# SyamVangara/multigrid-petsc

Hardware: AMD Instinct MI355X
Metric: fp64 DOF-updates/sec per V-cycle at 1024^3 (higher is better)
Workload: dtype f64

## Files before the change

multigrid_petsc_amd/csrc/mgk_kernels3.hip:

```cpp
#include "mgk_dev.hpp"
#include <type_traits>

struct J3dArgs {
    const double *u, *b, *uc;
    double *out;
    int nx, ny, nxc, nyc;
    long rs, crs;
    int ntx, yc, nwaves, xcd, bous, plainst;
    double a0, a2, a3, a4, a6, dinv, scale;
    const double *ctab, *dtab;
    double *partials;
    double *rout;
};
template <bool PRO, bool ZG, bool NORM, bool TAB, int YC>
__global__ void __launch_bounds__(256) k_jacobi3_2d(const J3dArgs a) {
    using VT = V16<double>;
    const int lane = threadIdx.x & 63;
    int bid = blockIdx.x;
    if (a.xcd) bid = (bid & 7) * (gridDim.x >> 3) + (bid >> 3);
    const int wid = __builtin_amdgcn_readfirstlane(bid * 4 + (threadIdx.x >> 6));
    const int tx = wid % a.ntx, cy = wid / a.ntx;
    const int yc = YC > 0 ? YC : a.yc;
    const int y0 = cy * yc, y1 = min(y0 + yc, a.ny);
    if (y0 >= y1) { if (NORM && lane == 0) a.partials[wid] = 0.0; return; }
    const int pidx = tx * 60 + lane - 2;
    const int x0 = 2 * pidx;
    const bool xin = (x0 >= 0 && x0 < a.nx);
    const bool lastvec = (x0 + 2 > a.nx);
    const bool store = (lane >= 2 && lane <= 61 && xin);
    const int xc = min(max(x0, 0), a.nx - 1);
    const double *__restrict__ up_ = a.u + xc;
    const double *__restrict__ bp_ = a.b + xc;
    const double *__restrict__ cp_ = PRO ? a.uc + min(max(pidx, -1), a.nxc) : nullptr;
    double *__restrict__ op_ = a.out + x0;
    const VT Z = v16_zero<double>();
    const bool nts = a.plainst == 2 || (a.plainst == 0 && mgk_store_nt_2d(a.ny, a.rs));
    auto fix = [&](VT v, int y) -> VT {
        if (!xin || y < 0 || y >= a.ny) { v.v[0] = 0.0; v.v[1] = 0.0; }
        if (lastvec) v.v[1] = 0.0;
        return v;
    };
    auto ldraw = [&](int y) -> VT { return *reinterpret_cast<const VT *>(up_ + (long)min(max(y, -1), a.ny) * a.rs); };
    auto ldbraw = [&](int y) -> VT { return ldv_stream(bp_ + (long)min(max(y, 0), a.ny - 1) * a.rs, true); };
    auto ldc = [&](int ic) -> double { return PRO ? cp_[(long)min(max(ic, -1), a.nyc) * a.crs] : 0.0; };
    auto pA = [&](int y) { return (y & 1) ? (y - 1) >> 1 : (y >> 1) - 1; };
    auto pB = [&](int y) { return (y & 1) ? (y - 1) >> 1 : (y >> 1); };
    auto correct = [&](VT v, int y, double cA, double cB) -> VT {
        if (PRO) {
            const bool two = ((y & 1) == 0);
            const double wi = two ? 0.5 : 1.0;
            const double wh = wi * 0.5, w1 = wi * 1.0;
            const double mA = lane_up<true>(cA), mB = lane_up<true>(cB);
            double s0 = 0.0, s1 = 0.0;
            s0 += wh * mA; s0 += wh * cA; s1 += w1 * cA;
            if (two) { s0 += wh * mB; s0 += wh * cB; s1 += w1 * cB; }
            v.v[0] = v.v[0] + s0; v.v[1] = v.v[1] + s1;
        }
        return fix(v, y);
    };
    struct K6 { double k0, k2, k3, k4, k6, kd; };
    auto ldk = [&](int y) -> K6 {
        K6 k = {a.a0, a.a2, a.a3, a.a4, a.a6, a.dinv};
        if (TAB) {
            const int yy_ = min(max(y, 0), a.ny - 1);
            const CDBL4 *cr_ = (const CDBL4 *)(a.ctab + 5 * (long)yy_);
            const CDBL4 *dr_ = (const CDBL4 *)(a.dtab + yy_);
            k.k0 = cr_[0]; k.k2 = cr_[1]; k.k3 = cr_[2]; k.k4 = cr_[3]; k.k6 = cr_[4]; k.kd = dr_[0];
        }
        return k;
    };
#define J3_COEFS(kk)                                                                                                  \
    const double k0 = TAB ? (kk).k0 : a.a0, k2 = TAB ? (kk).k2 : a.a2, k3 = TAB ? (kk).k3 : a.a3, k4 = TAB ? (kk).k4 : a.a4,    \
                 k6 = TAB ? (kk).k6 : a.a6, kd = TAB ? (kk).kd : a.dinv;
    double nacc = 0.0;
    auto sweep = [&](const VT &lo, const VT &c, const VT &hi, const VT &bb, int y, bool norm, const K6 &kk) -> VT {
        J3_COEFS(kk)
        const double Wv = lane_up<true>(c.v[1]), Ev = lane_dn<true>(c.v[0]);
        VT o, rr;
#pragma unroll
        for (int e = 0; e < 2; e++) {
            const double wv = (e == 0) ? Wv : c.v[0];
            const double ev = (e == 1) ? Ev : c.v[1];
            double s = k0 * lo.v[e];
            s = s + k2 * wv;
            s = s + k3 * c.v[e];
            s = s + k4 * ev;
            s = s + k6 * hi.v[e];
            const double res = bb.v[e] - s;
            const double zz = res * kd;
            o.v[e] = c.v[e] + a.scale * zz;
            rr.v[e] = (lastvec && e == 1) ? 0.0 : res;
            if (NORM && norm) nacc += (store && y >= y0 && y < y1 && !(lastvec && e == 1)) ? res * res : 0.0;
        }
        if (NORM && norm && a.rout && store && y >= y0 && y < y1) stv_policy(a.rout + (long)y * a.rs + x0, rr, nts);
        return fix(o, y);
    };
    auto sweep0 = [&](const VT &bb, int y, const K6 &kk) -> VT {
        J3_COEFS(kk)
        (void)k0; (void)k2; (void)k3; (void)k4; (void)k6;
        VT o;
#pragma unroll
        for (int e = 0; e < 2; e++) { const double zz = bb.v[e] * kd; o.v[e] = a.scale * zz; }
        return fix(o, y);
    };
    VT UU[2] = {Z, Z};
    VT BB[3] = {Z, Z, Z};
    VT PP[2] = {Z, Z};
    VT QQ[2] = {Z, Z};
    auto stepg = [&](auto revc, const int K, int t, const VT &ur, double cA, double cB, const VT &bnext) {
        constexpr bool REV = decltype(revc)::value;
        auto ph = [&](int tt) -> int { return REV ? (y0 + y1 - 1 - tt) : tt; };
        const K6 kc2 = ldk(ph(t + 2)), kc1 = ldk(ph(t + 1)), kc0 = ldk(ph(t));
        VT &ua = UU[K & 1], &ub = UU[(K + 1) & 1];
        VT &p0 = PP[K & 1], &p1 = PP[(K + 1) & 1];
        VT &q0 = QQ[K & 1], &q1 = QQ[(K + 1) & 1];
        VT &b0 = BB[K % 3], &b1 = BB[(K + 1) % 3], &b2 = BB[(K + 2) % 3];
        VT p2;
        if (ZG) p2 = sweep0(b2, ph(t + 2), kc2);
        else {
            const VT uc = correct(ur, ph(t + 3), cA, cB);
            p2 = REV ? sweep(uc, ub, ua, b2, ph(t + 2), true, kc2) : sweep(ua, ub, uc, b2, ph(t + 2), true, kc2);
            ua = uc;
        }
        if (t >= y0 - 2) {
            const VT q2 = REV ? sweep(p2, p1, p0, b1, ph(t + 1), false, kc1) : sweep(p0, p1, p2, b1, ph(t + 1), false, kc1);
            if (t >= y0 && t < y1) {
                const VT o = REV ? sweep(q2, q1, q0, b0, ph(t), false, kc0) : sweep(q0, q1, q2, b0, ph(t), false, kc0);
                if (store) stv_policy(op_ + (long)ph(t) * a.rs, o, nts);
            }
            q0 = q2;
        }
        p0 = p2;
        b0 = fix(bnext, ph(t + 3));
    };
    const int t0 = y0 - 4;
    if constexpr (YC > 0) {
        constexpr int NU = YC + 6, NC = NU / 2 + 2;
        VT U[NU], B[NU];
        double Cc[NC];
        const int c0 = pA(t0 + 1);
#pragma unroll
        for (int q = 0; q < NU; q++) { if (!ZG) U[q] = ldraw(t0 + 1 + q); B[q] = ldbraw(t0 + 1 + q); }
#pragma unroll
        for (int q = 0; q < NC; q++) Cc[q] = ldc(c0 + q);
        if (!ZG) {
            UU[0] = correct(U[0], t0 + 1, Cc[0], Cc[0]);
            UU[1] = correct(U[1], t0 + 2, Cc[0], Cc[1]);
        }
        BB[2] = fix(B[1], t0 + 2);
#pragma unroll
        for (int sidx = 0; sidx < YC + 4; sidx++) {
            const int k = sidx + 3;
            const int ia = (k & 1) ? (k - 1) / 2 : k / 2 - 1;
            const int ib = (k & 1) ? (k - 1) / 2 : k / 2;
            stepg(std::false_type{}, sidx % 6, t0 + sidx, ZG ? Z : U[sidx + 2], Cc[ia], Cc[ib], B[sidx + 2]);
        }
    } else {
        auto march = [&](auto revc) {
            constexpr bool REV = decltype(revc)::value;
            auto ph = [&](int tt) -> int { return REV ? (y0 + y1 - 1 - tt) : tt; };
            VT UR[2] = {Z, Z}, BN[2];
            double CA[2] = {0.0, 0.0}, CB[2] = {0.0, 0.0};
            if (!ZG) {
                UU[0] = correct(ldraw(ph(t0 + 1)), ph(t0 + 1), ldc(pA(ph(t0 + 1))), ldc(pB(ph(t0 + 1))));
                UU[1] = correct(ldraw(ph(t0 + 2)), ph(t0 + 2), ldc(pA(ph(t0 + 2))), ldc(pB(ph(t0 + 2))));
                UR[0] = ldraw(ph(t0 + 3));
                CA[0] = ldc(pA(ph(t0 + 3))); CB[0] = ldc(pB(ph(t0 + 3)));
            }
            BB[2] = fix(ldbraw(ph(t0 + 2)), ph(t0 + 2));
            BN[0] = ldbraw(ph(t0 + 3));
            auto S = [&](const int K, int t) {
                if (!ZG) { UR[(K + 1) & 1] = ldraw(ph(t + 4)); CA[(K + 1) & 1] = ldc(pA(ph(t + 4))); CB[(K + 1) & 1] = ldc(pB(ph(t + 4))); }
                BN[(K + 1) & 1] = ldbraw(ph(t + 4));
                stepg(revc, K, t, UR[K & 1], CA[K & 1], CB[K & 1], BN[K & 1]);
            };
            int t = t0;
            for (; t + 6 <= y1; t += 6) { S(0, t); S(1, t + 1); S(2, t + 2); S(3, t + 3); S(4, t + 4); S(5, t + 5); }
            if (t < y1) { S(0, t); t++; }
            if (t < y1) { S(1, t); t++; }
            if (t < y1) { S(2, t); t++; }
            if (t < y1) { S(3, t); t++; }
            if (t < y1) { S(4, t); t++; }
        };
        if (a.bous && ((cy & 1) || a.bous == 2)) march(std::true_type{}); else march(std::false_type{});
    }
    if (NORM) {
        const double sw = wave_sum(nacc);
        if (lane == 0) a.partials[wid] = sw;
    }
#undef J3_COEFS
}
template <bool PRO, bool ZG, bool NORM>
static int jacobi3_2d(mgk_ctx *c, const mgk_geom *g, const mgk_geom *gc, const double *coef, double dinv, double scale, const double *ctab, const double *dtab,
                      const double *b, const double *uc, const double *u, double *unew, void *stream, int *norm_parts, double *rout = nullptr) {
    if (!c || !g || g->dim != 2 || (!coef && !ctab) || (ctab && !dtab) || !b || !unew || (!ZG && (!u || u == unew)) || b == unew)
        return fail(MGK_EINVAL, "mgk_jacobi3_2d: bad arguments (2-D)");
    J3dArgs a; memset(&a, 0, sizeof(a));
    a.u = ZG ? nullptr : u + g->org; a.b = b + g->org; a.out = unew + g->org;
    a.nx = g->nx; a.ny = g->ny; a.rs = g->pitch;
    if (PRO) {
        if (!gc || !uc || gc->dim != 2 || g->nx != 2 * gc->nx + 1 || g->ny != 2 * gc->ny + 1) return fail(MGK_EINVAL, "mgk_prolong_jacobi3_2d: coarse grid does not match");
        a.uc = uc + gc->org; a.nxc = gc->nx; a.nyc = gc->ny; a.crs = gc->pitch;
    }
    if (coef) { a.a0 = coef[0]; a.a2 = coef[1]; a.a3 = coef[2]; a.a4 = coef[3]; a.a6 = coef[4]; }
    a.dinv = dinv; a.scale = scale; a.ctab = ctab; a.dtab = dtab;
    if (rout) { if (!NORM || rout == unew || rout == u || rout == b) return fail(MGK_EINVAL, "mgk_jacobi3_2d_sumsq_store_f64: bad arguments"); a.rout = rout + g->org; }
    a.ntx = ((g->nx + 1) / 2 + 59) / 60;
    int ycs = (g->nx + 1 <= 1024) ? 4 : 0;
    if (g_variant == 50) ycs = 0; else if (g_variant == 51) ycs = 4; else if (g_variant == 52) ycs = 8;
    if (g_zchunk > 0 && g_variant != 51 && g_variant != 52) ycs = 0;
    long nch = (4096 + a.ntx - 1) / a.ntx;
    if (g_zchunk > 0) nch = (g->ny + g_zchunk - 1) / g_zchunk;
    int yc = (int)((g->ny + nch - 1) / nch);
    if (yc < 12 && g_zchunk <= 0) yc = 12;
    if (yc > g->ny) yc = g->ny;
    if (ycs) yc = ycs;
    long waves = (long)a.ntx * ((g->ny + yc - 1) / yc);
    if (NORM && ((waves + 3) / 4 + 7) * 4 > c->max_partials) {
        if (ycs) { ycs = 0; }
        const long maxch = c->max_partials / a.ntx - 1;
        if (maxch < 1) return fail(MGK_EINVAL, "mgk_jacobi3_2d_sumsq_f64: more waves than partial slots");
        yc = (int)((g->ny + maxch - 1) / maxch);
        waves = (long)a.ntx * ((g->ny + yc - 1) / yc);
    }
    a.yc = yc;
    unsigned nblk = (unsigned)((waves + 3) / 4);
    a.xcd = (g_variant == 54) || (g_variant != 53 && nblk >= 64 && (ycs != 0 || g->nx >= 4095));
    if (a.xcd) nblk = (nblk + 7u) & ~7u;
    a.nwaves = (int)waves;
    a.bous = (ycs == 0 && g_variant == 58) ? 1 : (ycs == 0 && g_variant == 59) ? 2 : 0;
    a.plainst = (g_variant == 60) ? 1 : (g_variant == 61) ? 2 : 0;
    if (NORM) {
        if (!norm_parts || 4L * nblk > c->max_partials) return fail(MGK_EINVAL, "mgk_jacobi3_2d_sumsq_f64: more waves than partial slots");
        a.partials = c->partials;
        *norm_parts = (int)(4 * nblk);
    }
    hipStream_t st = S(c, stream);
#define J3_LAUNCH(TABV, YCV) hipLaunchKernelGGL((k_jacobi3_2d<PRO, ZG, NORM, TABV, YCV>), dim3(nblk), dim3(256), 0, st, a)
    if (ctab) { if (ycs == 4) J3_LAUNCH(true, 4); else if (ycs == 8) J3_LAUNCH(true, 8); else J3_LAUNCH(true, 0); }
    else { if (ycs == 4) J3_LAUNCH(false, 4); else if (ycs == 8) J3_LAUNCH(false, 8); else J3_LAUNCH(false, 0); }
#undef J3_LAUNCH
    HIPCHK(hipGetLastError());
    return 0;
}
extern "C" int mgk_jacobi3_2d_f64(mgk_ctx *c, const mgk_geom *g, const double *coef, double dinv, double scale, const double *ctab, const double *dtab,
                                  const double *b, const double *u, double *unew, void *stream) {
    return jacobi3_2d<false, false, false>(c, g, nullptr, coef, dinv, scale, ctab, dtab, b, nullptr, u, unew, stream, nullptr);
}
extern "C" int mgk_jacobi3_2d_sumsq_f64(mgk_ctx *c, const mgk_geom *g, const double *coef, double dinv, double scale, const double *ctab, const double *dtab,
                                        const double *b, const double *u, double *unew, double *sumsq_host, void *stream) {
    if (!sumsq_host) return fail(MGK_EINVAL, "mgk_jacobi3_2d_sumsq_f64: bad arguments");
    int nparts = 0;
    int rc = jacobi3_2d<false, false, true>(c, g, nullptr, coef, dinv, scale, ctab, dtab, b, nullptr, u, unew, stream, &nparts);
    if (rc) return rc;
    return finish_to_host(c, nparts, 1, S(c, stream), sumsq_host);
}
extern "C" int mgk_jacobi3_2d_sumsq_store_f64(mgk_ctx *c, const mgk_geom *g, const double *coef, double dinv, double scale, const double *ctab, const double *dtab,
                                              const double *b, const double *u, double *unew, double *r, double *sumsq_host, void *stream) {
    if (!sumsq_host || !r) return fail(MGK_EINVAL, "mgk_jacobi3_2d_sumsq_store_f64: bad arguments");
    int nparts = 0;
    int rc = jacobi3_2d<false, false, true>(c, g, nullptr, coef, dinv, scale, ctab, dtab, b, nullptr, u, unew, stream, &nparts, r);
    if (rc) return rc;
    return finish_to_host(c, nparts, 1, S(c, stream), sumsq_host);
}
extern "C" int mgk_jacobi3_2d_zero_f64(mgk_ctx *c, const mgk_geom *g, const double *coef, double dinv, double scale, const double *ctab, const double *dtab,
                                       const double *b, double *unew, void *stream) {
    return jacobi3_2d<false, true, false>(c, g, nullptr, coef, dinv, scale, ctab, dtab, b, nullptr, nullptr, unew, stream, nullptr);
}
extern "C" int mgk_prolong_jacobi3_2d_f64(mgk_ctx *c, const mgk_geom *gf, const mgk_geom *gc, const double *coef, double dinv, double scale,
                                          const double *ctab, const double *dtab, const double *b, const double *uc, const double *u, double *unew, void *stream) {
    return jacobi3_2d<true, false, false>(c, gf, gc, coef, dinv, scale, ctab, dtab, b, uc, u, unew, stream, nullptr);
}

struct J33Args {
    const double *u, *b;
    double *out;
    int nx, ny, nz;
    long rs, ms;
    int ntx, nty, ntz, zc, xcd;
    double a0, a1, a2, a3, a4, a5, a6, dinv, scale;
    double *partials;
};
template <int TY, bool NORM, int g_form>
__global__ void __launch_bounds__(256, 1) k_jacobi3_3d(const J33Args a) {
    constexpr int R0 = TY + 6, R1 = TY + 4, R2 = TY + 2;
    using VT = V16<double>;
    const int lane = threadIdx.x & 63;
    int bid = blockIdx.x;
    if (a.xcd) bid = (bid & 7) * (gridDim.x >> 3) + (bid >> 3);
    const int wid = bid * 4 + __builtin_amdgcn_readfirstlane((int)(threadIdx.x >> 6));
    const int tx = wid % a.ntx, ty = (wid / a.ntx) % a.nty, tz = wid / (a.ntx * a.nty);
    const int z0 = tz * a.zc, z1 = min(z0 + a.zc, a.nz);
    if (tz >= a.ntz || z0 >= z1) { if (NORM && lane == 0) a.partials[wid] = 0.0; return; }
    const int yb = ty * TY;
    const int x0 = 2 * (tx * 60 + lane - 2);
    const bool xin = (x0 >= 0 && x0 < a.nx);
    const bool lastvec = (x0 + 2 > a.nx);
    const bool store = (lane >= 2 && lane <= 61 && xin);
    const unsigned lo = (unsigned)(8 * min(x0, a.nx + 1));
    const char *__restrict__ ub_ = reinterpret_cast<const char *>(a.u);
    const char *__restrict__ bb_ = reinterpret_cast<const char *>(a.b);
    char *__restrict__ ob_ = reinterpret_cast<char *>(a.out);
    const long loff = (long)(int)lo;
    const VT Z = v16_zero<double>();
    long uro[R0], bro[R1];
#pragma unroll
    for (int r = 0; r < R0; r++) uro[r] = 8 * (long)min(max(yb - 3 + r, -1), a.ny) * a.rs;
#pragma unroll
    for (int q = 0; q < R1; q++) bro[q] = 8 * (long)min(max(yb - 2 + q, 0), a.ny - 1) * a.rs;
    bool rowok[R1];
#pragma unroll
    for (int q = 0; q < R1; q++) rowok[q] = (yb - 2 + q >= 0 && yb - 2 + q < a.ny);
    double nacc = 0.0;
    const unsigned long long Mx0 = xin ? ~0ull : 0ull, Mx1 = (xin && !lastvec) ? ~0ull : 0ull;
    auto andm = [](double v, unsigned long long m) -> double { return __longlong_as_double((long long)((unsigned long long)__double_as_longlong(v) & m)); };
    auto jac = [&](const VT &dn, const VT &sv, const VT &c, const VT &nv, const VT &upv, const VT &bb, unsigned long long mu, bool own, bool norm) -> VT {
        const double Wv = lane_up<true>(c.v[1]), Ev = lane_dn<true>(c.v[0]);
        VT o;
#pragma unroll
        for (int e = 0; e < 2; e++) {
            const double wv = (e == 0) ? Wv : c.v[0];
            const double ev = (e == 1) ? Ev : c.v[1];
            double s = a.a0 * dn.v[e];
            s = s + a.a1 * sv.v[e];
            s = s + a.a2 * wv;
            s = s + a.a3 * c.v[e];
            s = s + a.a4 * ev;
            s = s + a.a5 * nv.v[e];
            s = s + a.a6 * upv.v[e];
            const double res = bb.v[e] - s;
            const double zz = res * a.dinv;
            const double val = c.v[e] + a.scale * zz;
            const unsigned long long m = (e == 0 ? Mx0 : Mx1) & mu;
            o.v[e] = andm(val, m);
            if (NORM && norm) { const double rm = andm(res, (own && store) ? m : 0ull); nacc += rm * rm; }
        }
        return o;
    };
    auto ldplane = [&](VT (&P)[R0], int z) {
        const char *pz = ub_ + 8 * (long)min(max(z, -1), a.nz) * a.ms + loff;
#pragma unroll
        for (int r = 0; r < R0; r++) P[r] = *reinterpret_cast<const VT *>(pz + uro[r]);
    };
    auto ldb = [&](VT (&P)[R1], int z) {
        const char *pz = bb_ + 8 * (long)min(max(z, 0), a.nz - 1) * a.ms + loff;
#pragma unroll
        for (int q = 0; q < R1; q++) P[q] = ldv_stream(reinterpret_cast<const double *>(pz + bro[q]), true);
    };
#define J33_STAGE(NR, OUT, DN, o_dn, C, UP, o_up, BB, o_b, MASK, ...)                                            \
    {                                                                                                                  \
        double s_[NR][2], w_[NR], e_[NR];                                                                              \
        _Pragma("unroll") for (int q = 0; q < NR; q++) { w_[q] = lane_up<true>(C[q + 1].v[1]); e_[q] = lane_dn<true>(C[q + 1].v[0]); } \
        _Pragma("unroll") for (int q = 0; q < NR; q++) { s_[q][0] = a.a0 * DN[q + o_dn].v[0]; s_[q][1] = a.a0 * DN[q + o_dn].v[1]; } \
        _Pragma("unroll") for (int q = 0; q < NR; q++) { s_[q][0] = s_[q][0] + a.a1 * C[q].v[0]; s_[q][1] = s_[q][1] + a.a1 * C[q].v[1]; } \
        _Pragma("unroll") for (int q = 0; q < NR; q++) { s_[q][0] = s_[q][0] + a.a2 * w_[q]; s_[q][1] = s_[q][1] + a.a2 * C[q + 1].v[0]; } \
        _Pragma("unroll") for (int q = 0; q < NR; q++) { s_[q][0] = s_[q][0] + a.a3 * C[q + 1].v[0]; s_[q][1] = s_[q][1] + a.a3 * C[q + 1].v[1]; } \
        _Pragma("unroll") for (int q = 0; q < NR; q++) { s_[q][0] = s_[q][0] + a.a4 * C[q + 1].v[1]; s_[q][1] = s_[q][1] + a.a4 * e_[q]; } \
        _Pragma("unroll") for (int q = 0; q < NR; q++) { s_[q][0] = s_[q][0] + a.a5 * C[q + 2].v[0]; s_[q][1] = s_[q][1] + a.a5 * C[q + 2].v[1]; } \
        _Pragma("unroll") for (int q = 0; q < NR; q++) { s_[q][0] = s_[q][0] + a.a6 * UP[q + o_up].v[0]; s_[q][1] = s_[q][1] + a.a6 * UP[q + o_up].v[1]; } \
        _Pragma("unroll") for (int q = 0; q < NR; q++) {                                                               \
            const double r0_ = BB[q + o_b].v[0] - s_[q][0], r1_ = BB[q + o_b].v[1] - s_[q][1];                          \
            const double z0_ = r0_ * a.dinv, z1_ = r1_ * a.dinv;                                                       \
            const double v0_ = C[q + 1].v[0] + a.scale * z0_, v1_ = C[q + 1].v[1] + a.scale * z1_;                     \
            const unsigned long long mu_ = MASK;                                                                       \
            OUT[q].v[0] = andm(v0_, Mx0 & mu_); OUT[q].v[1] = andm(v1_, Mx1 & mu_);                                   \
            __VA_ARGS__                                                                                                \
        }                                                                                                              \
    }
    unsigned long long rowm[R1];
#pragma unroll
    for (int q = 0; q < R1; q++) rowm[q] = rowok[q] ? ~0ull : 0ull;
    const int t0 = z0 - 4;
    VT U[3][R0], Un[R0];
    VT P[3][R1];
    VT Q[3][R2];
    VT B[3][R1], Bn[R1];
    ldplane(U[0], t0 + 1); ldplane(U[1], t0 + 2); ldplane(U[2], t0 + 3);
    ldb(B[2], t0 + 2);
#pragma unroll
    for (int k = 0; k < 3; k++) {
#pragma unroll
        for (int q = 0; q < R1; q++) { P[k][q] = Z; if (k < 2) B[k][q] = Z; }
#pragma unroll
        for (int q = 0; q < R2; q++) Q[k][q] = Z;
    }
    auto step = [&](auto phc, int t) {
        constexpr int PH = decltype(phc)::value, S0 = PH % 3, S1 = (PH + 1) % 3, S2 = (PH + 2) % 3;
        ldplane(Un, t + 4);
        ldb(Bn, t + 3);
        const unsigned long long z2m = (t + 2 >= 0 && t + 2 < a.nz) ? ~0ull : 0ull, z1m = (t + 1 >= 0 && t + 1 < a.nz) ? ~0ull : 0ull;
        const bool z2own = (t + 2 >= z0 && t + 2 < z1);
        if (g_form == 0) {
#pragma unroll
        for (int q = 0; q < R1; q++)
            P[S2][q] = jac(U[S0][q + 1], U[S1][q], U[S1][q + 1], U[S1][q + 2], U[S2][q + 1], B[S2][q], rowm[q] & z2m, z2own && q >= 2 && q < 2 + TY, true);
        if (t >= z0 - 2) {
#pragma unroll
            for (int q = 0; q < R2; q++)
                Q[S2][q] = jac(P[S0][q + 1], P[S1][q], P[S1][q + 1], P[S1][q + 2], P[S2][q + 1], B[S1][q + 1], rowm[q + 1] & z1m, false, false);
            if (t >= z0) {
#pragma unroll
                for (int j = 0; j < TY; j++) {
                    const VT o = jac(Q[S0][j + 1], Q[S1][j], Q[S1][j + 1], Q[S1][j + 2], Q[S2][j + 1], B[S0][j + 2], ~0ull, false, false);
                    if (store && rowok[j + 2]) stv_stream(reinterpret_cast<double *>(ob_ + 8 * ((long)t * a.ms + (long)(yb + j) * a.rs) + loff), o);
                }
            }
        }
        } else {
        J33_STAGE(R1, P[S2], U[S0], 1, U[S1], U[S2], 1, B[S2], 0, (rowm[q] & z2m),
                  if (NORM) { const unsigned long long mn_ = (z2own && q >= 2 && q < 2 + TY && store) ? mu_ : 0ull;
                              const double n0_ = andm(r0_, Mx0 & mn_), n1_ = andm(r1_, Mx1 & mn_); nacc += n0_ * n0_; nacc += n1_ * n1_; })
        if (t >= z0 - 2) {
            J33_STAGE(R2, Q[S2], P[S0], 1, P[S1], P[S2], 1, B[S1], 1, (rowm[q + 1] & z1m), ;)
            if (t >= z0) {
                VT O[TY];
                J33_STAGE(TY, O, Q[S0], 1, Q[S1], Q[S2], 1, B[S0], 2, (~0ull), ;)
#pragma unroll
                for (int j = 0; j < TY; j++)
                    if (store && rowok[j + 2]) stv_stream(reinterpret_cast<double *>(ob_ + 8 * ((long)t * a.ms + (long)(yb + j) * a.rs) + loff), O[j]);
            }
        }
        }
#pragma unroll
        for (int r = 0; r < R0; r++) U[S0][r] = Un[r];
#pragma unroll
        for (int q = 0; q < R1; q++) B[S0][q] = Bn[q];
    };
    for (int t = t0; t < z1; t += 3) {
        step(std::integral_constant<int, 0>{}, t);
        if (t + 1 < z1) step(std::integral_constant<int, 1>{}, t + 1);
        if (t + 2 < z1) step(std::integral_constant<int, 2>{}, t + 2);
    }
    if (NORM) {
        const double sw = wave_sum(nacc);
        if (lane == 0) a.partials[wid] = sw;
    }
#undef J33_STAGE
}
template <int TY, bool NORM>
static int jacobi3_3d_launch(mgk_ctx *c, J33Args &a, const mgk_geom *g, int *norm_parts, void *stream) {
    a.ntx = ((g->nx + 1) / 2 + 59) / 60;
    a.nty = (g->ny + TY - 1) / TY;
    const long per = (long)a.ntx * a.nty;
    int ntz = 1;
    if (g_zchunk > 0) ntz = (g->nz + g_zchunk - 1) / g_zchunk;
    else { while (per * ntz < 4096 && g->nz / (ntz + 1) >= 32) ntz++; }
    if (NORM) while (ntz > 1 && per * ntz + 32 > c->max_partials) ntz--;
    a.zc = (g->nz + ntz - 1) / ntz;
    a.ntz = (g->nz + a.zc - 1) / a.zc;
    const long waves = per * a.ntz;
    unsigned nblk = (unsigned)((waves + 3) / 4);
    a.xcd = (g_variant != 53 && nblk >= 64) ? 1 : 0;
    if (a.xcd) nblk = (nblk + 7u) & ~7u;
    if (NORM) {
        if (!norm_parts || 4L * nblk > c->max_partials) return fail(MGK_EINVAL, "mgk_jacobi3_sumsq_f64: more waves than partial slots");
        a.partials = c->partials;
        *norm_parts = (int)(4 * nblk);
    }
    if (g_variant == 64) hipLaunchKernelGGL((k_jacobi3_3d<TY, NORM, 0>), dim3(nblk), dim3(256), 0, S(c, stream), a);
    else hipLaunchKernelGGL((k_jacobi3_3d<TY, NORM, 1>), dim3(nblk), dim3(256), 0, S(c, stream), a);
    HIPCHK(hipGetLastError());
    return 0;
}
template <bool NORM>
static int jacobi3_3d(mgk_ctx *c, const mgk_geom *g, const double *coef, double dinv, double scale, const double *b, const double *u, double *unew,
                      void *stream, int *norm_parts) {
    if (!c || !g || g->dim != 3 || !coef || !b || !u || !unew || u == unew || b == unew) return fail(MGK_EINVAL, "mgk_jacobi3_f64: bad arguments (3-D)");
    J33Args a; memset(&a, 0, sizeof(a));
    a.u = u + g->org; a.b = b + g->org; a.out = unew + g->org;
    a.nx = g->nx; a.ny = g->ny; a.nz = g->nz; a.rs = g->pitch; a.ms = g->plane;
    a.a0 = coef[0]; a.a1 = coef[1]; a.a2 = coef[2]; a.a3 = coef[3]; a.a4 = coef[4]; a.a5 = coef[5]; a.a6 = coef[6];
    a.dinv = dinv; a.scale = scale;
    const int ty = (g_variant == 62) ? 2 : (g_variant == 63 || NORM) ? 3 : 4;
    if (ty == 2) return jacobi3_3d_launch<2, NORM>(c, a, g, norm_parts, stream);
    if (ty == 3) return jacobi3_3d_launch<3, NORM>(c, a, g, norm_parts, stream);
    return jacobi3_3d_launch<4, NORM>(c, a, g, norm_parts, stream);
}
extern "C" int mgk_jacobi3_f64(mgk_ctx *c, const mgk_geom *g, const double *coef, double dinv, double scale,
                               const double *b, const double *u, double *unew, void *stream) {
    return jacobi3_3d<false>(c, g, coef, dinv, scale, b, u, unew, stream, nullptr);
}
extern "C" int mgk_jacobi3_sumsq_f64(mgk_ctx *c, const mgk_geom *g, const double *coef, double dinv, double scale,
                                     const double *b, const double *u, double *unew, double *sumsq_host, void *stream) {
    if (!sumsq_host) return fail(MGK_EINVAL, "mgk_jacobi3_sumsq_f64: bad arguments");
    int nparts = 0;
    int rc = jacobi3_3d<true>(c, g, coef, dinv, scale, b, u, unew, stream, &nparts);
    if (rc) return rc;
    return finish_to_host(c, nparts, 1, S(c, stream), sumsq_host);
}

extern "C" int mgk_ipc_alloc(mgk_ctx *c, size_t bytes, void **ptr, void *handle64) {
    if (!c || !ptr || !handle64 || !bytes) return fail(MGK_EINVAL, "mgk_ipc_alloc: bad arguments");
    HIPCHK(hipSetDevice(c->device));
    HIPCHK(hipExtMallocWithFlags(ptr, bytes, hipDeviceMallocFinegrained));
    HIPCHK(hipMemsetAsync(*ptr, 0, bytes, c->compute));
    HIPCHK(hipStreamSynchronize(c->compute));
    hipIpcMemHandle_t h;
    HIPCHK(hipIpcGetMemHandle(&h, *ptr));
    static_assert(sizeof(h) == MGK_IPC_HANDLE_BYTES, "handle size");
    memcpy(handle64, &h, sizeof(h));
    return 0;
}
extern "C" int mgk_ipc_open(mgk_ctx *c, const void *handle64, void **ptr) {
    if (!c || !ptr || !handle64) return fail(MGK_EINVAL, "mgk_ipc_open: bad arguments");
    HIPCHK(hipSetDevice(c->device));
    hipIpcMemHandle_t h;
    memcpy(&h, handle64, sizeof(h));
    HIPCHK(hipIpcOpenMemHandle(ptr, h, hipIpcMemLazyEnablePeerAccess));
    return 0;
}
extern "C" int mgk_ipc_close(mgk_ctx *c, void *ptr) { (void)c; if (ptr) HIPCHK(hipIpcCloseMemHandle(ptr)); return 0; }
extern "C" int mgk_peer_copy(mgk_ctx *c, void *dst, const void *src, size_t bytes, void *stream) {
    if (!c || !dst || !src) return fail(MGK_EINVAL, "mgk_peer_copy: bad arguments");
    if (bytes) HIPCHK(hipMemcpyAsync(dst, src, bytes, hipMemcpyDefault, S(c, stream)));
    return 0;
}
struct FlagArgs { unsigned long long *flag[MGK_PEER_MAX]; int n; unsigned long long value, ticks; unsigned int *status; };
__global__ void __launch_bounds__(64) k_flag_set(const FlagArgs a) {
    if ((int)threadIdx.x < a.n) __hip_atomic_store(a.flag[threadIdx.x], a.value, __ATOMIC_RELEASE, __HIP_MEMORY_SCOPE_SYSTEM);
}
__global__ void __launch_bounds__(64) k_flag_wait(const FlagArgs a) {
    if ((int)threadIdx.x >= a.n) return;
    const unsigned long long t0 = __builtin_amdgcn_s_memrealtime();
    while (__hip_atomic_load(a.flag[threadIdx.x], __ATOMIC_ACQUIRE, __HIP_MEMORY_SCOPE_SYSTEM) < a.value) {
        if (__builtin_amdgcn_s_memrealtime() - t0 > a.ticks) { __hip_atomic_store(a.status, 1u, __ATOMIC_RELAXED, __HIP_MEMORY_SCOPE_SYSTEM); return; }
        __builtin_amdgcn_s_sleep(16);
    }
}
static int flag_args(FlagArgs &a, void *const *flags, int n, unsigned long long value) {
    memset(&a, 0, sizeof(a));
    if (!flags || n < 1 || n > MGK_PEER_MAX) return 1;
    for (int q = 0; q < n; q++) { if (!flags[q]) return 1; a.flag[q] = (unsigned long long *)flags[q]; }
    a.n = n; a.value = value;
    return 0;
}
extern "C" int mgk_flags_set(mgk_ctx *c, void *const *flags, int n, unsigned long long value, void *stream) {
    FlagArgs a;
    if (!c || flag_args(a, flags, n, value)) return fail(MGK_EINVAL, "mgk_flags_set: bad arguments");
    hipLaunchKernelGGL(k_flag_set, dim3(1), dim3(64), 0, S(c, stream), a);
    HIPCHK(hipGetLastError());
    return 0;
}
extern "C" int mgk_flags_wait(mgk_ctx *c, void *const *flags, int n, unsigned long long value, double timeout_s, void *status_u32, void *stream) {
    FlagArgs a;
    if (!c || !status_u32 || !(timeout_s > 0.0) || flag_args(a, flags, n, value)) return fail(MGK_EINVAL, "mgk_flags_wait: bad arguments");
    a.ticks = (unsigned long long)(timeout_s * 1.0e8); a.status = (unsigned int *)status_u32;
    hipLaunchKernelGGL(k_flag_wait, dim3(1), dim3(64), 0, S(c, stream), a);
    HIPCHK(hipGetLastError());
    return 0;
}
int mgk_preload_kernels3() {
    hipFuncAttributes fa;
    HIPCHK(hipFuncGetAttributes(&fa, reinterpret_cast<const void *>(k_flag_set)));
    return 0;
}
extern "C" int mgk_flag_set(mgk_ctx *c, void *flag, unsigned long long value, void *stream) { void *f[1] = {flag}; return mgk_flags_set(c, f, 1, value, stream); }
extern "C" int mgk_flag_wait(mgk_ctx *c, const void *flag, unsigned long long value, double timeout_s, void *status_u32, void *stream) {
    void *f[1] = {const_cast<void *>(flag)};
    return mgk_flags_wait(c, f, 1, value, timeout_s, status_u32, stream);
}
struct ARArgs { unsigned long long *peers[MGK_PEER_MAX]; int nranks, me, n; unsigned long long seq, ticks; double *vals; unsigned int *status; };
__global__ void __launch_bounds__(64) k_peer_allreduce(const ARArgs a) {
    const int lane = threadIdx.x;
    const int buf = (int)(a.seq & 1ull);
    const double mine = lane < a.n ? a.vals[lane] : 0.0;
    for (int r = 0; r < a.nranks; r++) {
        unsigned long long *slot = a.peers[r] + 65 * (buf * a.nranks + a.me);
        if (lane < a.n) __hip_atomic_store(reinterpret_cast<double *>(slot + 1 + lane), mine, __ATOMIC_RELAXED, __HIP_MEMORY_SCOPE_SYSTEM);
    }
    __builtin_amdgcn_fence(__ATOMIC_RELEASE, "");
    __builtin_amdgcn_s_waitcnt(0);
    if (lane == 0) for (int r = 0; r < a.nranks; r++) __hip_atomic_store(a.peers[r] + 65 * (buf * a.nranks + a.me), a.seq, __ATOMIC_RELEASE, __HIP_MEMORY_SCOPE_SYSTEM);
    const unsigned long long *own = a.peers[a.me] + 65 * buf * a.nranks;
    const unsigned long long t0 = __builtin_amdgcn_s_memrealtime();
    bool ok = true;
    if (lane < a.nranks) {
        while (__hip_atomic_load(own + 65 * lane, __ATOMIC_ACQUIRE, __HIP_MEMORY_SCOPE_SYSTEM) < a.seq) {
            if (__builtin_amdgcn_s_memrealtime() - t0 > a.ticks) { ok = false; break; }
            __builtin_amdgcn_s_sleep(16);
        }
    }
    if (!ok) __hip_atomic_store(a.status, 1u, __ATOMIC_RELAXED, __HIP_MEMORY_SCOPE_SYSTEM);
    __builtin_amdgcn_fence(__ATOMIC_ACQUIRE, "");
    if (lane < a.n) {
        double s = 0.0;
        for (int r = 0; r < a.nranks; r++) s += __hip_atomic_load(reinterpret_cast<const double *>(own + 65 * r + 1 + lane), __ATOMIC_RELAXED, __HIP_MEMORY_SCOPE_SYSTEM);
        a.vals[lane] = s;
    }
}
extern "C" int mgk_peer_allreduce(mgk_ctx *c, void *const *peer_blocks, int nranks, int me, unsigned long long seq, double *vals_dev, int n,
                                  double timeout_s, void *status_u32, void *stream) {
    if (!c || !peer_blocks || nranks < 1 || nranks > MGK_PEER_MAX || me < 0 || me >= nranks || !vals_dev || n < 1 || n > 64 || !status_u32)
        return fail(MGK_EINVAL, "mgk_peer_allreduce: bad arguments");
    ARArgs a; memset(&a, 0, sizeof(a));
    for (int r = 0; r < nranks; r++) { if (!peer_blocks[r]) return fail(MGK_EINVAL, "mgk_peer_allreduce: unmapped peer"); a.peers[r] = (unsigned long long *)peer_blocks[r]; }
    a.nranks = nranks; a.me = me; a.n = n; a.seq = seq; a.ticks = (unsigned long long)(timeout_s * 1.0e8); a.vals = vals_dev; a.status = (unsigned int *)status_u32;
    hipLaunchKernelGGL(k_peer_allreduce, dim3(1), dim3(64), 0, S(c, stream), a);
    HIPCHK(hipGetLastError());
    return 0;
}
```

Measured before the change: 383.3 billion.

## Add LDS-tiled 3-sweep temporal-blocked Jacobi kernel as default 3-D smoother

Result: no change. 386.0 billion, median of 6 (+0.7%).

```diff
diff --git a/multigrid_petsc_amd/csrc/mgk_kernels3.hip b/multigrid_petsc_amd/csrc/mgk_kernels3.hip
--- a/multigrid_petsc_amd/csrc/mgk_kernels3.hip
+++ b/multigrid_petsc_amd/csrc/mgk_kernels3.hip
@@ -437,6 +437,175 @@
     }
 #undef J33_STAGE
 }
+typedef unsigned int mgk_u2v __attribute__((ext_vector_type(2)));
+template <bool NORM, int D>
+__global__ void __launch_bounds__(512) k_jacobi3_tile(const J33Args a) {
+    constexpr int R = 3 + D;
+    constexpr int NT = 512, TXO = 64, TYO = 32, UW = TXO + 6, UH = TYO + 6, NPT = UW * UH, NS = (NPT + NT - 1) / NT, SB = NS * NT;
+    constexpr int LU = 0, LS1 = 2, LS2 = 4;
+    __shared__ double lds_[6 * SB + 2 * UW];
+    double *const lds = lds_ + UW;
+    const int tid = threadIdx.x;
+    const int w = __builtin_amdgcn_readfirstlane(tid >> 6);
+    int bid = blockIdx.x;
+    if (a.xcd) bid = (bid & 7) * (gridDim.x >> 3) + (bid >> 3);
+    const int tx = bid % a.ntx, ty = (bid / a.ntx) % a.nty, tz = bid / (a.ntx * a.nty);
+    const int z0 = tz * a.zc, z1 = min(z0 + a.zc, a.nz);
+    if (tz >= a.ntz || z0 >= z1) { if (NORM && tid == 0) a.partials[blockIdx.x] = 0.0; return; }
+    const int xb = tx * TXO - 3, yb = ty * TYO - 3;
+
+    unsigned off[NS];
+    unsigned mg[NS];
+    bool own[NS];
+#pragma unroll
+    for (int k = 0; k < NS; k++) {
+        const int f = tid + NT * k;
+        const int lx = f < NPT ? f % UW : 0, ly = f < NPT ? f / UW : 0;
+        const int x = xb + lx, y = yb + ly;
+        const bool in = f < NPT && x >= 0 && x < a.nx && y >= 0 && y < a.ny;
+        mg[k] = in ? ~0u : 0u;
+        own[k] = in && lx >= 3 && lx < UW - 3 && ly >= 3 && ly < UH - 3;
+        off[k] = 8u * (unsigned)((min(max(y, -1), a.ny) + 1) * a.rs + (min(max(x, -1), a.nx) + 1));
+    }
+    auto live = [&](int k) { return NT * k + 64 * w < NPT; };
+    auto rows_reach = [](int k, int s) { return (NT * k) / UW < UH - s && (NT * k + NT - 1) / UW >= s; };
+    const int pbytes = (int)(8 * a.ms);
+    auto prs = [&](const double *f, int z) {
+        return __builtin_amdgcn_make_buffer_rsrc((void *)(f - a.rs - 1 + (long)min(max(z, -1), a.nz) * a.ms), 0, pbytes, 0x00020000);
+    };
+    auto ld = [](__amdgpu_buffer_rsrc_t r, unsigned o) { return __builtin_bit_cast(double, __builtin_amdgcn_raw_buffer_load_b64(r, o, 0, 0)); };
+    auto andm = [](double v, unsigned m) -> double {
+        const unsigned long long m2 = ((unsigned long long)m << 32) | m;
+        return __longlong_as_double((long long)((unsigned long long)__double_as_longlong(v) & m2));
+    };
+    auto jac = [&](double dn, double sv, double wv, double c, double ev, double nv, double upv, double bv, double &res) -> double {
+        double s = a.a0 * dn;
+        s = s + a.a1 * sv;
+        s = s + a.a2 * wv;
+        s = s + a.a3 * c;
+        s = s + a.a4 * ev;
+        s = s + a.a5 * nv;
+        s = s + a.a6 * upv;
+        res = bv - s;
+        const double zz = res * a.dinv;
+        return c + a.scale * zz;
+    };
+
+    double U[R][NS], B[R][NS], S1m[NS], S1c[NS], S2m[NS], S2c[NS];
+    double nacc = 0.0;
+    const int t0 = z0 - 4;
+    {
+#pragma unroll
+        for (int k = 0; k < NS; k++) {
+#pragma unroll
+            for (int r = 0; r < R; r++) {
+                U[r][k] = r < R - 1 ? ld(prs(a.u, t0 + 1 + r), off[k]) : 0.0;
+                B[r][k] = r >= 2 && r < R - 1 ? ld(prs(a.b, t0 + r), off[k]) : 0.0;
+            }
+            S1m[k] = S1c[k] = S2m[k] = S2c[k] = 0.0;
+            lds[(LU + ((t0 + 2) & 1)) * SB + tid + NT * k] = U[1][k];
+        }
+    }
+    __syncthreads();
+
+    auto step = [&](auto ph, const int t) __attribute__((always_inline)) {
+        constexpr int PH = decltype(ph)::value;
+        constexpr int IM = PH % R, IC = (PH + 1) % R, IP = (PH + 2) % R, IN = (PH + R - 1) % R;
+        {
+            const auto un = prs(a.u, t + R), bn = prs(a.b, t + R - 1);
+#pragma unroll
+            for (int k = 0; k < NS; k++) { U[IN][k] = ld(un, off[k]); B[IN][k] = ld(bn, off[k]); }
+        }
+        const unsigned m1 = (t + 2 >= 0 && t + 2 < a.nz) ? ~0u : 0u, m2 = (t + 1 >= 0 && t + 1 < a.nz) ? ~0u : 0u;
+        const bool nrm = NORM && t + 2 >= z0 && t + 2 < z1;
+        double S1p[NS], S2p[NS];
+#pragma unroll
+        for (int k = 0; k < NS; k++) S2p[k] = 0.0;
+        {
+            const double *L = lds + (LU + ((t + 2) & 1)) * SB + tid;
+            double *O = lds + (LS1 + ((t + 2) & 1)) * SB + tid;
+#pragma unroll
+            for (int k = 0; k < NS; k++) {
+                S1p[k] = 0.0;
+                if (live(k)) {
+                    double res;
+                    const double v = jac(U[IM][k], L[NT * k - UW], L[NT * k - 1], U[IC][k], L[NT * k + 1], L[NT * k + UW], U[IP][k], B[IP][k], res);
+                    S1p[k] = andm(v, mg[k] & m1);
+                    O[NT * k] = S1p[k];
+                    if (nrm) { const double rm = andm(res, own[k] ? mg[k] : 0u); nacc += rm * rm; }
+                }
+            }
+        }
+        if (t >= z0 - 2) {
+            const double *L = lds + (LS1 + ((t + 1) & 1)) * SB + tid;
+            double *O = lds + (LS2 + ((t + 1) & 1)) * SB + tid;
+#pragma unroll
+            for (int k = 0; k < NS; k++) {
+                if (rows_reach(k, 2) && live(k)) {
+                    double res;
+                    const double v = jac(S1m[k], L[NT * k - UW], L[NT * k - 1], S1c[k], L[NT * k + 1], L[NT * k + UW], S1p[k], B[IC][k], res);
+                    S2p[k] = andm(v, mg[k] & m2);
+                    O[NT * k] = S2p[k];
+                }
+            }
+            if (t >= z0) {
+                const double *L = lds + (LS2 + (t & 1)) * SB + tid;
+                const auto out = prs(a.out, t);
+#pragma unroll
+                for (int k = 0; k < NS; k++) {
+                    if (rows_reach(k, 3) && live(k)) {
+                        double res;
+                        const double v = jac(S2m[k], L[NT * k - UW], L[NT * k - 1], S2c[k], L[NT * k + 1], L[NT * k + UW], S2p[k], B[IM][k], res);
+                        if (own[k]) __builtin_amdgcn_raw_buffer_store_b64(__builtin_bit_cast(mgk_u2v, v), out, off[k], 0, 2);
+                    }
+                }
+            }
+        }
+        {
+            double *O = lds + (LU + ((t + 3) & 1)) * SB + tid;
+#pragma unroll
+            for (int k = 0; k < NS; k++) if (live(k)) O[NT * k] = U[IP][k];
+        }
+        __syncthreads();
+#pragma unroll
+        for (int k = 0; k < NS; k++) { S1m[k] = S1c[k]; S1c[k] = S1p[k]; S2m[k] = S2c[k]; S2c[k] = S2p[k]; }
+    };
+    for (int t = t0; t < z1; t += R) {
+        step(std::integral_constant<int, 0>{}, t);
+        if (t + 1 < z1) step(std::integral_constant<int, 1>{}, t + 1);
+        if (t + 2 < z1) step(std::integral_constant<int, 2>{}, t + 2);
+        if (t + 3 < z1) step(std::integral_constant<int, 3>{}, t + 3);
+        if (R > 4 && t + 4 < z1) step(std::integral_constant<int, 4 % R>{}, t + 4);
+    }
+    if (NORM) {
+        const double sblk = block_sum(nacc, lds_);
+        if (tid == 0) a.partials[blockIdx.x] = sblk;
+    }
+}
+template <bool NORM>
+static int jacobi3_tile_launch(mgk_ctx *c, J33Args &a, const mgk_geom *g, int *norm_parts, void *stream) {
+    a.ntx = (g->nx + 63) / 64;
+    a.nty = (g->ny + 31) / 32;
+    const long per = (long)a.ntx * a.nty;
+    int ntz = 1;
+    if (g_zchunk > 0) ntz = (g->nz + g_zchunk - 1) / g_zchunk;
+    else { while (per * ntz < 1024 && g->nz / (ntz + 1) >= 16) ntz++; }
+    if (NORM) while (ntz > 1 && per * ntz + 8 > c->max_partials) ntz--;
+    a.zc = (g->nz + ntz - 1) / ntz;
+    a.ntz = (g->nz + a.zc - 1) / a.zc;
+    unsigned nblk = (unsigned)(per * a.ntz);
+    a.xcd = (g_variant != 53 && nblk >= 64) ? 1 : 0;
+    if (a.xcd) nblk = (nblk + 7u) & ~7u;
+    if (NORM) {
+        if (!norm_parts || (long)nblk > c->max_partials) return fail(MGK_EINVAL, "mgk_jacobi3_sumsq_f64: more blocks than partial slots");
+        a.partials = c->partials;
+        *norm_parts = (int)nblk;
+    }
+    if (!NORM && g_variant == 66) hipLaunchKernelGGL((k_jacobi3_tile<NORM, 2>), dim3(nblk), dim3(512), 0, S(c, stream), a);
+    else hipLaunchKernelGGL((k_jacobi3_tile<NORM, 1>), dim3(nblk), dim3(512), 0, S(c, stream), a);
+    HIPCHK(hipGetLastError());
+    return 0;
+}
 template <int TY, bool NORM>
 static int jacobi3_3d_launch(mgk_ctx *c, J33Args &a, const mgk_geom *g, int *norm_parts, void *stream) {
     a.ntx = ((g->nx + 1) / 2 + 59) / 60;
@@ -471,6 +640,7 @@
     a.nx = g->nx; a.ny = g->ny; a.nz = g->nz; a.rs = g->pitch; a.ms = g->plane;
     a.a0 = coef[0]; a.a1 = coef[1]; a.a2 = coef[2]; a.a3 = coef[3]; a.a4 = coef[4]; a.a5 = coef[5]; a.a6 = coef[6];
     a.dinv = dinv; a.scale = scale;
+    if (g_variant < 62 || g_variant > 65) return jacobi3_tile_launch<NORM>(c, a, g, norm_parts, stream);
     const int ty = (g_variant == 62) ? 2 : (g_variant == 63 || NORM) ? 3 : 4;
     if (ty == 2) return jacobi3_3d_launch<2, NORM>(c, a, g, norm_parts, stream);
     if (ty == 3) return jacobi3_3d_launch<3, NORM>(c, a, g, norm_parts, stream);
```
